# ivan-digital/qwen3-asr-swift

Hardware: NVIDIA B200
Metric: RTFx (audio-sec/sec) Qwen3-ASR-0.6B batched (higher is better)
Workload: dtype bf16

## Files before the change

### qwen3-asr-swift_b200/csrc/api.cu

```cuda
#include <stdio.h>
#include <string.h>

#include <algorithm>
#include <mutex>

#include "gemm.cuh"
#include "model.h"

using namespace q3;

struct q3asr_handle {
    Handle h;
};

namespace {

thread_local std::string g_create_error;

template <typename F>
int guarded(q3asr_handle* hh, F&& fn) {
    if (hh == nullptr) return Q3ASR_ERR_INVALID;
    try {
        DeviceGuard g(hh->h.device);
        fn(hh->h);
// ... 675 lines not shown
        Q3_H2D_SYNC(dseg, seg_row0, sizeof(int) * n_segs);
        Q3_H2D_SYNC(dseg + n_segs, seg_len, sizeof(int) * n_segs);
        Q3_CUDA(cudaMemset(dout, 0, 2 * nq));
        int max_len = 0;
        for (int i = 0; i < n_segs; i++) max_len = std::max(max_len, seg_len[i]);
        AttnSegs segs{dseg, dseg + n_segs, n_segs, max_len};
        cudaError_t se = cudaSuccess;
        try {
            const int ldq = heads * head_dim, ldk = (heads / group) * head_dim;
            if (kernel == 0)
                flash_attn_tc_launch(dq, ldq, dk, ldk, dv, ldk, dout, ldq, segs, rows, heads, group, head_dim, causal != 0, scale, h.stream);
            else
                flash_attn_launch(dq, ldq, dk, ldk, dv, ldk, dout, ldq, segs, heads, group, head_dim, causal != 0, scale, h.stream);
            se = cudaStreamSynchronize(h.stream);
            if (se == cudaSuccess) se = cudaMemcpy(out, dout, 2 * nq, cudaMemcpyDeviceToHost);
        } catch (...) {
            cudaFree(dq); cudaFree(dk); cudaFree(dv); cudaFree(dout); cudaFree(dseg);
            throw;
        }
        cudaFree(dq); cudaFree(dk); cudaFree(dv); cudaFree(dout); cudaFree(dseg);
        Q3_CUDA(se);
    });
}

int q3asr_debug_decode_attention(q3asr_handle* hh, const float* qkv_part, int splits, int n_seqs, int heads, int kv_heads,
                                 const uint16_t* q_norm, const uint16_t* k_norm, float eps, float scale, const int* kv_len,
                                 const int* page_table, int max_pages, uint16_t* pool, int n_pages, int layers, int layer, int variant,
                                 int launches, uint16_t* out) {
    return guarded(hh, [&](Handle& h) {
        Q3_CHECK(h.loaded && h.model, Q3ASR_ERR_STATE, "debug_decode_attention: no model loaded (the RoPE frequencies come from it)");
        Q3_CHECK(qkv_part && q_norm && k_norm && kv_len && page_table && pool && out && splits >= 1 && n_seqs >= 1 && kv_heads >= 1 &&
                     heads >= 1 && max_pages >= 1 && n_pages >= 1 && layers >= 1 && layer >= 0 && layer < layers && launches >= 1,
                 Q3ASR_ERR_INVALID, "debug_decode_attention: bad argument");
        Q3_CHECK(variant == -1 || variant == 0 || variant == 1 || variant == 2 || variant == 4 || variant == 8 || variant == 16,
                 Q3ASR_ERR_INVALID, "debug_decode_attention: variant must be -1, 0, 1, 2, 4, 8 or 16");
        Q3_CHECK(variant == -1 ? (heads == kv_heads || heads == 2 * kv_heads) : heads == 2 * kv_heads, Q3ASR_ERR_INVALID,
                 "debug_decode_attention: the fused kernels take 2 query heads per kv head, the general path 1 or 2");
        for (size_t i = 0; i < (size_t)n_seqs * max_pages; i++)
            Q3_CHECK(page_table[i] >= 0 && page_table[i] < n_pages, Q3ASR_ERR_INVALID, "debug_decode_attention: page-table entry out of range");
        for (int s = 0; s < n_seqs; s++)
            Q3_CHECK(kv_len[s] >= 1 && kv_len[s] <= max_pages * KV_PAGE, Q3ASR_ERR_INVALID, "debug_decode_attention: kv_len out of range");
        const int nqkv = (heads + 2 * kv_heads) * 128, n_pos = max_pages * KV_PAGE;
        const size_t part_n = (size_t)splits * n_seqs * nqkv, out_n = (size_t)n_seqs * heads * 128;
        const size_t pool_n = (size_t)n_pages * layers * 2 * kv_heads * KV_PAGE * 128;
        DebugAllocs a;
        std::vector<int> pos(n_seqs), row_seq(n_seqs);
        for (int s = 0; s < n_seqs; s++) { pos[s] = kv_len[s] - 1; row_seq[s] = s; }
        float* dpart = a.get<float>(part_n);
        bf16 *dqw = a.get<bf16>(128), *dkw = a.get<bf16>(128), *dpool = a.get<bf16>(pool_n), *dout = a.get<bf16>(out_n * launches);
        int *dlen = a.get<int>(n_seqs), *dpos = a.get<int>(n_seqs), *dpt = a.get<int>((size_t)n_seqs * max_pages);
        float2* drope = a.get<float2>((size_t)n_pos * 64);
        Q3_H2D_SYNC(dpart, qkv_part, sizeof(float) * part_n);
        Q3_H2D_SYNC(dqw, q_norm, 2 * 128);
        Q3_H2D_SYNC(dkw, k_norm, 2 * 128);
        Q3_H2D_SYNC(dpool, pool, 2 * pool_n);
        Q3_H2D_SYNC(dlen, kv_len, sizeof(int) * n_seqs);
        Q3_H2D_SYNC(dpos, pos.data(), sizeof(int) * n_seqs);
        Q3_H2D_SYNC(dpt, page_table, sizeof(int) * (size_t)n_seqs * max_pages);
        rope_table_launch(h.model->inv_freq, n_pos, drope, nullptr, h.stream);
        const KvCache cache{dpool, dpt, max_pages, layers, kv_heads, 128};
        if (variant == -1) {
            std::vector<bf16> qkv((size_t)n_seqs * nqkv);
            for (size_t i = 0; i < qkv.size(); i++) {
                float acc = 0.f;
                for (int sp = 0; sp < splits; sp++) acc += qkv_part[(size_t)sp * n_seqs * nqkv + i];
                qkv[i] = __float2bfloat16_rn(acc);
            }
            bf16 *dqkv = a.get<bf16>(qkv.size()), *dq = a.get<bf16>(out_n);
// ... 96 lines not shown
```

### qwen3-asr-swift_b200/csrc/gemm.cu

```cuda
#include <cudaTypedefs.h>
#include <stdlib.h>

#include <atomic>
#include <vector>

#include "gemm2.cuh"
#include "lmhead.cuh"
#include "skinny.cuh"

namespace q3 {

namespace {

PFN_cuTensorMapEncodeTiled_v12000 g_encode = nullptr;
int g_num_sms = 148;
thread_local unsigned long long g_launches = 0;

void make_tmap(CUtensorMap* m, const void* ptr, int rank, const cuuint64_t* dims, const cuuint64_t* strides_bytes,
               const cuuint32_t* box, const cuuint32_t* estr, CUtensorMapSwizzle swizzle = CU_TENSOR_MAP_SWIZZLE_128B) {
    Q3_CHECK(g_encode != nullptr, 2, "gemm_init() has not been called");
    CUresult r = g_encode(m, CU_TENSOR_MAP_DATA_TYPE_BFLOAT16, (cuuint32_t)rank, const_cast<void*>(ptr), dims, strides_bytes, box,
                          estr, CU_TENSOR_MAP_INTERLEAVE_NONE, swizzle, CU_TENSOR_MAP_L2_PROMOTION_L2_256B,
                          CU_TENSOR_MAP_FLOAT_OOB_FILL_NONE);
    if (r != CUDA_SUCCESS) {
        std::string s = "cuTensorMapEncodeTiled failed (" + std::to_string((int)r) + "): rank " + std::to_string(rank) + " dims";
        for (int i = 0; i < rank; i++) s += " " + std::to_string((unsigned long long)dims[i]);
        s += " strides";
        for (int i = 0; i + 1 < rank; i++) s += " " + std::to_string((unsigned long long)strides_bytes[i]);
        s += " box";
        for (int i = 0; i < rank; i++) s += " " + std::to_string(box[i]);
        s += " estr";
        for (int i = 0; i < rank; i++) s += " " + std::to_string(estr[i]);
        throw Error(3, s);
    }
}

template <int BN, int EPI>
void launch_tc(const CUtensorMap& ta, const CUtensorMap& tb, const CUtensorMap& tc, GemmDev p, int max_stages, int grid, cudaStream_t st) {
    static PerDeviceOnce attr_once;
// ... 209 lines not shown
        s_m = mm;
    }
    __syncthreads();
    const float M = s_m;
    float s = 0.f;
    for (int t = threadIdx.x; t < tiles; t += blockDim.x) {
        const float mt = mx[t];
        if (mt != -INFINITY) s += sm[t] * __expf(mt - M);
    }
#pragma unroll
    for (int o = 16; o > 0; o >>= 1) s += __shfl_xor_sync(0xffffffffu, s, o);
    __syncthreads();
    if (lane == 0) sv[warp] = s;
    __syncthreads();
    if (threadIdx.x == 0) {
        float tot = 0.f;
        for (int w = 0; w < 8; w++) tot += sv[w];
        const float z = raw ? __bfloat162float(raw[(size_t)row * ld + bi]) : best;
        out[row] = bi;
        if (out_val) out_val[row] = best;
        out_lp[row] = (z - M) - logf(tot);
    }
}

}

void make_tmap_2d_bf16(CUtensorMap* m, const void* ptr, uint64_t cols, uint64_t rows, uint64_t row_stride_elems, uint32_t box_cols,
                       uint32_t box_rows) {
    cuuint64_t dims[2] = {(cuuint64_t)cols, (cuuint64_t)rows};
    cuuint64_t str[1] = {(cuuint64_t)row_stride_elems * 2};
    cuuint32_t box[2] = {box_cols, box_rows};
    cuuint32_t es[2] = {1, 1};
    make_tmap(m, ptr, 2, dims, str, box, es);
}

void gemm_init(int device) {
    if (g_encode == nullptr) {
        void* fn = nullptr;
        cudaDriverEntryPointQueryResult qres;
        Q3_CUDA(cudaGetDriverEntryPoint("cuTensorMapEncodeTiled", &fn, cudaEnableDefault, &qres));
        Q3_CHECK(qres == cudaDriverEntryPointSuccess && fn != nullptr, 3, "cuTensorMapEncodeTiled not available in this driver");
        g_encode = reinterpret_cast<PFN_cuTensorMapEncodeTiled_v12000>(fn);
    }
    cudaDeviceProp prop;
    Q3_CUDA(cudaGetDeviceProperties(&prop, device));
    Q3_CHECK(prop.major == 10, 3, std::string("q3asr kernels are built for sm_100a only; device is sm_") + std::to_string(prop.major) +
                                      std::to_string(prop.minor));
    g_num_sms = prop.multiProcessorCount;
}

int gemm_pick_bn(int N, int epi, long m_tiles) {
    static const int cand[] = {256, 224, 160, 128, 64, 32};
    int smallest = 0;
    for (int bn : cand) {
        if (N % bn) continue;
        if (epi == EPI_SWIGLU && bn % (2 * GU_UNIT)) continue;
        smallest = bn;
        if (m_tiles * (N / bn) >= 2L * g_num_sms) return bn;
    }
    Q3_CHECK(smallest != 0, 1, "gemm: N = " + std::to_string(N) + " is not a multiple of 32");
    return smallest;
}
int gemm_pick_bn(int N, int epi) { return gemm_pick_bn(N, epi, 1L << 20); }

void gemm_conv(const GemmA& a, const GemmShape& s, const bf16* W, int N, const GemmEpiArgs& e, cudaStream_t st, bool simt, int bn) {
    Q3_CHECK(a.C % 8 == 0 && a.C > 0, 1, "gemm: channel count must be a positive multiple of 8");
// ... 271 lines not shown
```

### qwen3-asr-swift_b200/csrc/ops.cu

```cuda
#include <stdlib.h>

#include <algorithm>

#include "ops.cuh"
#include "ptx.cuh"

namespace q3 {

namespace {

__device__ __forceinline__ uint2 ld8(const bf16* p) { return *reinterpret_cast<const uint2*>(p); }
__device__ __forceinline__ void st8(bf16* p, float a, float b, float c, float d) {
    *reinterpret_cast<uint2*>(p) = make_uint2(pack_bf16x2(a, b), pack_bf16x2(c, d));
}

__global__ void __launch_bounds__(256) conv1_kernel(const float* __restrict__ mel, const Conv1Chunk* __restrict__ chunks,
                                                    const bf16* __restrict__ w, const bf16* __restrict__ bias, int C, int chunk_w,
                                                    bf16* __restrict__ out) {
    extern __shared__ float2 s_in[];
    const int oh = blockIdx.x, g = blockIdx.y;
    const Conv1Chunk c = chunks[g];
    const int pitch = chunk_w + 2;
    for (int i = threadIdx.x; i < 3 * pitch; i += blockDim.x) {
        const int r = i / pitch, j = i % pitch - 1;
// ... 484 lines not shown
        out[((size_t)seq * heads + kvh * GROUP + g) * 128 + d] = __float2bfloat16_rn(num / den);
    }
}

constexpr int DM_CHUNK = 16;
constexpr int DM_STAGES = 3;
constexpr int DM_STREAMS = 8;

__device__ __forceinline__ float dm_merge_scales(float am, float bm, float* fa, float* fb) {
    const float m = fmaxf(am, bm);
    *fa = am == -INFINITY ? 0.f : exp2f(am - m);
    *fb = bm == -INFINITY ? 0.f : exp2f(bm - m);
    return m;
}
constexpr int decode_attn_mma_smem(int nw) { return nw * DM_STAGES * 2 * DM_CHUNK * 128 * 2; }

__device__ __forceinline__ void ldsm_x4(uint32_t (&r)[4], const void* smem_ptr) {
    const uint32_t a = static_cast<uint32_t>(__cvta_generic_to_shared(smem_ptr));
    asm volatile("ldmatrix.sync.aligned.m8n8.x4.shared.b16 {%0,%1,%2,%3}, [%4];" : "=r"(r[0]), "=r"(r[1]), "=r"(r[2]), "=r"(r[3]) : "r"(a));
}
__device__ __forceinline__ void ldsm_x4_t(uint32_t (&r)[4], const void* smem_ptr) {
    const uint32_t a = static_cast<uint32_t>(__cvta_generic_to_shared(smem_ptr));
    asm volatile("ldmatrix.sync.aligned.m8n8.x4.trans.shared.b16 {%0,%1,%2,%3}, [%4];"
                 : "=r"(r[0]), "=r"(r[1]), "=r"(r[2]), "=r"(r[3])
                 : "r"(a));
}
__device__ __forceinline__ void mma16816(float (&d)[4], const uint32_t (&a)[4], uint32_t b0, uint32_t b1) {
    asm volatile("mma.sync.aligned.m16n8k16.row.col.f32.bf16.bf16.f32 {%0,%1,%2,%3}, {%4,%5,%6,%7}, {%8,%9}, {%0,%1,%2,%3};"
                 : "+f"(d[0]), "+f"(d[1]), "+f"(d[2]), "+f"(d[3])
                 : "r"(a[0]), "r"(a[1]), "r"(a[2]), "r"(a[3]), "r"(b0), "r"(b1));
}
__device__ __forceinline__ int dm_off(int key, int seg) { return key * 128 + ((seg ^ (key & 7)) << 3); }

constexpr int DM_PART_STRIDE = 264;
template <int NW, bool SPLIT>
__global__ void __launch_bounds__(NW * 32, SPLIT ? 8 : NW == 2 ? 4 : 1) decode_attn_mma_kernel(const float* __restrict__ qkv_part, int splits, long long split_stride,
                                                                  int nqkv, const bf16* __restrict__ qw, const bf16* __restrict__ kw,
                                                                  const int* __restrict__ pos, float eps,
                                                                  const float2* __restrict__ rope_tab, KvCache cache, int layer,
                                                                  const int* __restrict__ kv_len, int heads, float scale_log2,
                                                                  bf16* __restrict__ out, float* __restrict__ split_part, int* __restrict__ split_cnt) {
    static_assert(!SPLIT || NW == 1, "the split variant is one warp per CTA");
    constexpr int GROUP = 2;
    constexpr int SW = SPLIT ? 2 : NW;
    ptx::grid_dep_launch();
    const int seq = blockIdx.x, kvh = blockIdx.y;
    const int lane = threadIdx.x & 31, warp = threadIdx.x >> 5;
    const int half = SPLIT ? (int)blockIdx.z : 0;
    const int sw0 = SPLIT ? half : warp;
    __shared__ __align__(16) bf16 s_qb[GROUP][128];
    __shared__ __align__(16) bf16 s_new[2][128];
    __shared__ float s_m[GROUP][NW], s_l[GROUP][NW];
    __shared__ float s_acc[GROUP][NW][128];
    const int* pt = cache.page_table + (size_t)seq * cache.max_pages;

    const int len = kv_len[seq];
    extern __shared__ uint4 da_smem[];
    bf16* ring = reinterpret_cast<bf16*>(da_smem) + (size_t)warp * DM_STAGES * 2 * DM_CHUNK * 128;
    const size_t head_off = (((size_t)layer * 2) * cache.kv_heads + kvh) * (KV_PAGE * 128);
    const size_t page_elems = (size_t)cache.layers * 2 * cache.kv_heads * (KV_PAGE * 128);
    const size_t v_off = (size_t)cache.kv_heads * (KV_PAGE * 128);
    const int n_chunks = (len + DM_CHUNK - 1) / DM_CHUNK;
    auto issue = [&](int chunk, int stage) {
        if (chunk < n_chunks) {
            const int j0 = chunk * DM_CHUNK;
            const bf16* kb = cache.pool + (size_t)pt[j0 / KV_PAGE] * page_elems + head_off + (j0 % KV_PAGE) * 128;
            bf16* sk = ring + (size_t)stage * 2 * DM_CHUNK * 128;
#pragma unroll
            for (int i = 0; i < DM_CHUNK * 16 / 32; i++) {
                const int lin = i * 32 + lane, key = lin >> 4, seg = lin & 15;
                const uint32_t n = j0 + key < len ? 16u : 0u;
                cp_async16(sk + dm_off(key, seg), kb + lin * 8, n);
                cp_async16(sk + DM_CHUNK * 128 + dm_off(key, seg), kb + v_off + lin * 8, n);
            }
        }
        asm volatile("cp.async.commit_group;" ::: "memory");
    };
    auto seq_next = [&](int& sj, int& sc) {
        sc += DM_STREAMS;
        while (sc >= n_chunks && sj + SW < DM_STREAMS) {
            sj += SW;
            sc = sj;
        }
    };
    int ij = sw0, ic = sw0;
    while (ic >= n_chunks && ij + SW < DM_STREAMS) { ij += SW; ic = ij; }
#pragma unroll
    for (int s = 0; s < DM_STAGES - 1; s++) {
        issue(ic, s);
        seq_next(ij, ic);
    }

    ptx::grid_dep_wait();

    const bool need_kv = !SPLIT || half == 0 || (((n_chunks - 1) % DM_STREAMS) & 1) == half;
    for (int vt = threadIdx.x; vt < 16 * (GROUP + 2) && (vt < 16 * GROUP || need_kv); vt += NW * 32) {
        const int slot = vt >> 4, hl = vt & 15;
        const unsigned half_mask = 0xffffu << (threadIdx.x & 16);
        const int d0 = hl * 8;
        const int col = slot < GROUP ? (kvh * GROUP + slot) * 128
                                     : slot == GROUP ? heads * 128 + kvh * 128 : (heads + cache.kv_heads) * 128 + kvh * 128;
        const float* src = qkv_part + (size_t)seq * nqkv + col + d0;
        float x[8] = {0.f, 0.f, 0.f, 0.f, 0.f, 0.f, 0.f, 0.f};
        for (int s0 = 0; s0 < splits; s0 += 4) {
            float4 b[4][2];
#pragma unroll
            for (int i = 0; i < 4; i++) {
                const bool on = s0 + i < splits;
                const float4* sp = reinterpret_cast<const float4*>(src + (size_t)(s0 + i) * split_stride);
                b[i][0] = on ? sp[0] : make_float4(0.f, 0.f, 0.f, 0.f);
                b[i][1] = on ? sp[1] : make_float4(0.f, 0.f, 0.f, 0.f);
            }
#pragma unroll
            for (int i = 0; i < 4; i++) {
                x[0] += b[i][0].x; x[1] += b[i][0].y; x[2] += b[i][0].z; x[3] += b[i][0].w;
                x[4] += b[i][1].x; x[5] += b[i][1].y; x[6] += b[i][1].z; x[7] += b[i][1].w;
            }
        }
#pragma unroll
        for (int j = 0; j < 8; j++) x[j] = bf16_round(x[j]);
        const int p = pos[seq];
        if (slot <= GROUP) {
            float q = 0.f;
#pragma unroll
            for (int j = 0; j < 8; j++) q = fmaf(x[j], x[j], q);
#pragma unroll
            for (int o = 8; o > 0; o >>= 1) q += __shfl_xor_sync(half_mask, q, o);
            const float r = rsqrtf(q * (1.0f / 128.0f) + eps);
            const uint4 wu = *reinterpret_cast<const uint4*>((slot < GROUP ? qw : kw) + d0);
            const uint32_t ww[4] = {wu.x, wu.y, wu.z, wu.w};
#pragma unroll
            for (int j = 0; j < 4; j++) {
                const float2 wf = unpack_bf16x2(ww[j]);
                x[2 * j] = bf16_round(x[2 * j] * r * wf.x);
                x[2 * j + 1] = bf16_round(x[2 * j + 1] * r * wf.y);
            }
            float y[8];
#pragma unroll
            for (int j = 0; j < 8; j++) y[j] = __shfl_xor_sync(half_mask, x[j], 8);
            const float sgn = hl < 8 ? -1.f : 1.f;
            const float4* tp = reinterpret_cast<const float4*>(rope_tab + (size_t)p * 64 + (d0 & 63));
#pragma unroll
            for (int j = 0; j < 4; j++) {
                const float4 t = __ldg(tp + j);
                x[2 * j] = fmaf(x[2 * j], t.x, sgn * y[2 * j] * t.y);
                x[2 * j + 1] = fmaf(x[2 * j + 1], t.z, sgn * y[2 * j + 1] * t.w);
            }
        }
        const uint4 packed = make_uint4(pack_bf16x2(x[0], x[1]), pack_bf16x2(x[2], x[3]), pack_bf16x2(x[4], x[5]), pack_bf16x2(x[6], x[7]));
        if (slot < GROUP) {
            *reinterpret_cast<uint4*>(&s_qb[slot][d0]) = packed;
        } else {
            const int page = pt[p / KV_PAGE];
            bf16* dst = cache.pool + ((((size_t)page * cache.layers + layer) * 2 + (slot == GROUP ? 0 : 1)) * cache.kv_heads + kvh) * (KV_PAGE * 128) +
                        (p % KV_PAGE) * 128 + d0;
            if (half == 0) *reinterpret_cast<uint4*>(dst) = packed;
            *reinterpret_cast<uint4*>(&s_new[slot - GROUP][d0]) = packed;
        }
    }
    __syncthreads();

    const int g = lane >> 2, t = lane & 3;
    uint32_t qa[8][2];
#pragma unroll
    for (int ks = 0; ks < 8; ks++) {
        qa[ks][0] = lane < 8 ? *reinterpret_cast<const uint32_t*>(&s_qb[g & 1][ks * 16 + t * 2]) : 0u;
        qa[ks][1] = lane < 8 ? *reinterpret_cast<const uint32_t*>(&s_qb[g & 1][ks * 16 + 8 + t * 2]) : 0u;
    }
    float o[16][4];
    float m_run = -INFINITY, l_run = 0.f;
    const int mi = lane >> 3, r8 = lane & 7;
    int stage = 0;
    int cj = sw0, chunk = sw0;
    while (chunk >= n_chunks && cj + SW < DM_STREAMS) { cj += SW; chunk = cj; }
    int cur_stream = -1;
    bool first_stream = true;
    auto flush_stream = [&]() {
        float l = l_run;
        l += __shfl_xor_sync(0xffffffffu, l, 1);
        l += __shfl_xor_sync(0xffffffffu, l, 2);
        if (lane < 8) {
            float am = first_stream ? -INFINITY : s_m[g][warp], al = first_stream ? 0.f : s_l[g][warp];
            float fa, fb;
            const float mm = dm_merge_scales(am, m_run, &fa, &fb);
#pragma unroll
            for (int nt = 0; nt < 16; nt++) {
                float* dst = &s_acc[g][warp][nt * 8 + t * 2];
                const float a0 = first_stream ? 0.f : dst[0], a1 = first_stream ? 0.f : dst[1];
                dst[0] = fmaf(fb, o[nt][0], fa * a0);
                dst[1] = fmaf(fb, o[nt][1], fa * a1);
            }
            __syncwarp(0xffu);
            if (t == 0) { s_m[g][warp] = mm; s_l[g][warp] = fmaf(fb, l, fa * al); }
        }
        first_stream = false;
    };
    for (; chunk < n_chunks; seq_next(cj, chunk)) {
        if (cj != cur_stream) {
            if (cur_stream >= 0) flush_stream();
            cur_stream = cj;
#pragma unroll
            for (int i = 0; i < 16; i++) o[i][0] = o[i][1] = o[i][2] = o[i][3] = 0.f;
            m_run = -INFINITY;
            l_run = 0.f;
        }
        issue(ic, (stage + DM_STAGES - 1) % DM_STAGES);
        seq_next(ij, ic);
        asm volatile("cp.async.wait_group %0;" ::"n"(DM_STAGES - 1) : "memory");
        __syncwarp();
        bf16* sk = ring + (size_t)stage * 2 * DM_CHUNK * 128;
        bf16* sv = sk + DM_CHUNK * 128;
        const int j0 = chunk * DM_CHUNK;
        if (chunk == n_chunks - 1) {
            const int row = (len - 1) - j0;
            *reinterpret_cast<uint4*>((lane < 16 ? sk : sv) + dm_off(row, lane & 15)) = reinterpret_cast<const uint4*>(s_new[lane >> 4])[lane & 15];
            __syncwarp();
        }
        float s[2][4];
#pragma unroll
        for (int i = 0; i < 2; i++) s[i][0] = s[i][1] = s[i][2] = s[i][3] = 0.f;
#pragma unroll
        for (int ks = 0; ks < 8; ks++) {
            uint32_t b[4];
            const int key = (mi >> 1) * 8 + r8;
            ldsm_x4(b, sk + dm_off(key, ks * 2 + (mi & 1)));
            const uint32_t a[4] = {qa[ks][0], 0u, qa[ks][1], 0u};
            mma16816(s[0], a, b[0], b[1]);
            mma16816(s[1], a, b[2], b[3]);
        }
        float mx = -INFINITY;
#pragma unroll
        for (int nt = 0; nt < 2; nt++)
#pragma unroll
            for (int e = 0; e < 2; e++) {
                const bool ok = j0 + nt * 8 + t * 2 + e < len;
                s[nt][e] = ok ? s[nt][e] * scale_log2 : -INFINITY;
                mx = fmaxf(mx, s[nt][e]);
            }
        mx = fmaxf(mx, __shfl_xor_sync(0xffffffffu, mx, 1));
        mx = fmaxf(mx, __shfl_xor_sync(0xffffffffu, mx, 2));
        const float mn = fmaxf(m_run, mx);
        const float alpha = exp2f(m_run - mn);
        m_run = mn;
        const float p00 = exp2f(s[0][0] - mn), p01 = exp2f(s[0][1] - mn), p10 = exp2f(s[1][0] - mn), p11 = exp2f(s[1][1] - mn);
        l_run = l_run * alpha + ((p00 + p01) + (p10 + p11));
        const uint32_t pa[4] = {pack_bf16x2(p00, p01), 0u, pack_bf16x2(p10, p11), 0u};
#pragma unroll
        for (int i = 0; i < 16; i++) { o[i][0] *= alpha; o[i][1] *= alpha; }
#pragma unroll
        for (int np = 0; np < 8; np++) {
            uint32_t b[4];
            const int key = r8 + (mi & 1) * 8;
            ldsm_x4_t(b, sv + dm_off(key, np * 2 + (mi >> 1)));
            mma16816(o[2 * np], pa, b[0], b[1]);
            mma16816(o[2 * np + 1], pa, b[2], b[3]);
        }
        __syncwarp();
        stage = (stage + 1) % DM_STAGES;
    }
    asm volatile("cp.async.wait_group 0;" ::: "memory");

    if (cur_stream >= 0) {
        flush_stream();
    } else if (lane < 8) {
        if (t == 0) { s_m[g][warp] = -INFINITY; s_l[g][warp] = 0.f; }
#pragma unroll
        for (int nt = 0; nt < 16; nt++) s_acc[g][warp][nt * 8 + t * 2] = s_acc[g][warp][nt * 8 + t * 2 + 1] = 0.f;
    }
    __syncthreads();
    if constexpr (SPLIT) {
        const size_t item = (size_t)seq * gridDim.y + kvh;
        float* mine = split_part + (item * 2 + half) * DM_PART_STRIDE;
        for (int i = lane; i < GROUP * 128; i += 32) mine[i] = s_acc[i >> 7][0][i & 127];
        if (lane < 2 * GROUP) mine[GROUP * 128 + lane] = lane < GROUP ? s_m[lane][0] : s_l[lane - GROUP][0];
        __threadfence();
        __syncwarp();
        int arrived = 0;
        if (lane == 0) arrived = atomicAdd(split_cnt + item, 1);
        arrived = __shfl_sync(0xffffffffu, arrived, 0);
        if (arrived == 0) return;
        __threadfence();
        const float* other = split_part + (item * 2 + (half ^ 1)) * DM_PART_STRIDE;
        for (int i = lane; i < GROUP * 128; i += 32) {
            const int gg = i >> 7, d = i & 127;
            const float om = __ldcg(other + GROUP * 128 + gg), ol = __ldcg(other + GROUP * 128 + GROUP + gg), oa = __ldcg(other + i);
            const float em = half == 0 ? s_m[gg][0] : om, el = half == 0 ? s_l[gg][0] : ol, ea = half == 0 ? s_acc[gg][0][d] : oa;
            const float dm = half == 0 ? om : s_m[gg][0], dl = half == 0 ? ol : s_l[gg][0], da = half == 0 ? oa : s_acc[gg][0][d];
            float fa, fb;
            dm_merge_scales(em, dm, &fa, &fb);
            const float num = fmaf(fb, da, fa * ea), den = fmaf(fb, dl, fa * el);
            out[((size_t)seq * heads + kvh * GROUP + gg) * 128 + d] = __float2bfloat16_rn(num / den);
        }
        if (lane == 0) split_cnt[item] = 0;
    } else
    for (int i = threadIdx.x; i < GROUP * 128; i += NW * 32) {
        const int gg = i >> 7, d = i & 127;
        float cm[2] = {-INFINITY, -INFINITY}, cl[2] = {0.f, 0.f}, ca[2] = {0.f, 0.f};
#pragma unroll
        for (int w = 0; w < NW; w++) {
            float fa, fb;
            const float mm = dm_merge_scales(cm[w & 1], s_m[gg][w], &fa, &fb);
            ca[w & 1] = fmaf(fb, s_acc[gg][w][d], fa * ca[w & 1]);
            cl[w & 1] = fmaf(fb, s_l[gg][w], fa * cl[w & 1]);
            cm[w & 1] = mm;
        }
        float fa, fb;
        dm_merge_scales(cm[0], cm[1], &fa, &fb);
        const float num = fmaf(fb, ca[1], fa * ca[0]), den = fmaf(fb, cl[1], fa * cl[0]);
        out[((size_t)seq * heads + kvh * GROUP + gg) * 128 + d] = __float2bfloat16_rn(num / den);
    }
}

__global__ void __launch_bounds__(1024) reduce_resid_rmsnorm_kernel(const float* __restrict__ part, int splits, long long split_stride,
                                                                    bf16* __restrict__ x, const bf16* __restrict__ w, bf16* __restrict__ y,
                                                                    int d, float eps) {
    ptx::grid_dep_launch();
    ptx::grid_dep_wait();
    __shared__ float4 s_part[1024];
    __shared__ float s_red[32];
    const int ncg = d >> 2, sg_count = blockDim.x / ncg;
    const int row = blockIdx.x, cg = threadIdx.x % ncg, sg = threadIdx.x / ncg, c0 = cg * 4;
    const float* src = part + (size_t)row * d + c0;
    float4 b[4];
#pragma unroll
    for (int i = 0; i < 4; i++) {
        const int sp = sg + i * sg_count;
        b[i] = sp < splits ? *reinterpret_cast<const float4*>(src + (size_t)sp * split_stride) : make_float4(0.f, 0.f, 0.f, 0.f);
    }
    float4 a = b[0];
#pragma unroll
    for (int i = 1; i < 4; i++) { a.x += b[i].x; a.y += b[i].y; a.z += b[i].z; a.w += b[i].w; }
    for (int sp = sg + 4 * sg_count; sp < splits; sp += sg_count) {
        const float4 t = *reinterpret_cast<const float4*>(src + (size_t)sp * split_stride);
        a.x += t.x; a.y += t.y; a.z += t.z; a.w += t.w;
    }
    s_part[threadIdx.x] = a;
    __syncthreads();
    float v[4] = {0.f, 0.f, 0.f, 0.f};
    float q = 0.f;
    if (sg == 0) {
        for (int g = 1; g < sg_count; g++) {
            const float4 t = s_part[g * ncg + cg];
// ... 337 lines not shown
    if (rows <= 0) return;
    launch_kernel(embed_splice_kernel, blocks_for((size_t)rows * (h / 8), 256), 256, 0, st, ids, audio_src, embed, audio, x, rows, h);
}

void qknorm_rope_kv_launch(const bf16* qkv, int ld, const bf16* qw, const bf16* kw, const int* pos, const int* row_seq, int rows,
                           int heads, int kv_heads, float eps, const float2* rope_tab, bf16* qout, bf16* kc, bf16* vc,
                           const KvCache& cache, int layer, cudaStream_t st) {
    if (rows <= 0) return;
    Q3_CHECK(cache.head_dim == 128, 1, "decoder head_dim must be 128");
    qknorm_rope_kv_kernel<<<rows, 256, 0, st>>>(qkv, ld, qw, kw, pos, row_seq, rows, heads, kv_heads, eps, rope_tab, qout,
                                                                kc, vc, cache, layer);
    Q3_CUDA(cudaGetLastError());
}

void rope_table_launch(const float* inv_freq, int n_pos, float2* tab, float2* tab_t, cudaStream_t st) {
    if (n_pos > 0) rope_table_kernel<<<blocks_for((size_t)n_pos * 64, 256), 256, 0, st>>>(inv_freq, n_pos, tab, tab_t);
    Q3_CUDA(cudaGetLastError());
}

void decode_attn_launch(const bf16* q, const KvCache& cache, int layer, const int* kv_len, int n_seqs, int heads, float scale, bf16* out,
                        cudaStream_t st) {
    if (n_seqs <= 0) return;
    const int group = heads / cache.kv_heads;
    const float sl2 = scale * 1.4426950408889634f;
    dim3 grid(n_seqs, cache.kv_heads);
    switch (group) {
        case 1: decode_attn_kernel<1><<<grid, 128, 0, st>>>(q, cache, layer, kv_len, heads, sl2, out); break;
        case 2: decode_attn_kernel<2><<<grid, 128, 0, st>>>(q, cache, layer, kv_len, heads, sl2, out); break;
        default: throw Error(1, "decode attention: only 1 or 2 query heads per kv head are built");
    }
    Q3_CUDA(cudaGetLastError());
}

void decode_attn_fused_launch(const float* qkv_part, int splits, long long split_stride, int nqkv, const bf16* qw, const bf16* kw,
                              const int* pos, float eps, const float2* rope_tab, const KvCache& cache, int layer, const int* kv_len,
                              int n_seqs, int heads, float scale, bf16* out, int num_sms, cudaStream_t st, float* split_part, int* split_cnt,
                              int force) {
    if (n_seqs <= 0) return;
    Q3_CHECK(cache.head_dim == 128, 1, "decoder head_dim must be 128");
    Q3_CHECK(heads == 2 * cache.kv_heads, 1, "fused decode attention is built for 2 query heads per kv head");
    Q3_CHECK(force == 0 || force == 2 || force == 4 || force == 8 || force == 16 || (force == 1 && split_part != nullptr && split_cnt != nullptr), 1,
             "fused decode attention: unknown variant");
    const float sl2 = scale * 1.4426950408889634f;
    dim3 grid(n_seqs, cache.kv_heads);
    static PerDeviceOnce attr_once;
    attr_once([] {
        Q3_CUDA(cudaFuncSetAttribute(decode_attn_fused_kernel<2, 4>, cudaFuncAttributeMaxDynamicSharedMemorySize, decode_attn_smem(4)));
        Q3_CUDA(cudaFuncSetAttribute(decode_attn_fused_kernel<2, 16>, cudaFuncAttributeMaxDynamicSharedMemorySize, decode_attn_smem(16)));
        Q3_CUDA(cudaFuncSetAttribute(decode_attn_mma_kernel<1, true>, cudaFuncAttributeMaxDynamicSharedMemorySize, decode_attn_mma_smem(1)));
        Q3_CUDA(cudaFuncSetAttribute(decode_attn_mma_kernel<2, false>, cudaFuncAttributeMaxDynamicSharedMemorySize, decode_attn_mma_smem(2)));
        Q3_CUDA(cudaFuncSetAttribute(decode_attn_mma_kernel<8, false>, cudaFuncAttributeMaxDynamicSharedMemorySize, decode_attn_mma_smem(8)));
    });
    const long items = (long)n_seqs * cache.kv_heads;
    int warps = items >= 2L * num_sms ? 2 : 8;
    if (const char* f = getenv("Q3ASR_DECODE_ATTN_WARPS")) {
        const int w = atoi(f);
        if (w == 2 || w == 8 || (w == 1 && split_part != nullptr && split_cnt != nullptr)) warps = w;
    }
    static const bool simt_env = getenv("Q3ASR_DECODE_ATTN_SIMT") != nullptr && atoi(getenv("Q3ASR_DECODE_ATTN_SIMT")) != 0;
    bool simt = simt_env;
    if (force != 0) {
        simt = force == 4 || force == 16;
        warps = force == 16 ? 8 : force == 4 ? 2 : force;
    }
    if (!simt) {
        if (warps == 1)
            launch_kernel(decode_attn_mma_kernel<1, true>, dim3(n_seqs, cache.kv_heads, 2), 32, decode_attn_mma_smem(1), st, qkv_part, splits,
                          split_stride, nqkv, qw, kw, pos, eps, rope_tab, cache, layer, kv_len, heads, sl2, out, split_part, split_cnt);
        else if (warps == 2)
            launch_kernel(decode_attn_mma_kernel<2, false>, grid, 64, decode_attn_mma_smem(2), st, qkv_part, splits, split_stride, nqkv, qw, kw, pos, eps,
                          rope_tab, cache, layer, kv_len, heads, sl2, out, split_part, split_cnt);
        else
            launch_kernel(decode_attn_mma_kernel<8, false>, grid, 256, decode_attn_mma_smem(8), st, qkv_part, splits, split_stride, nqkv, qw, kw, pos, eps,
                          rope_tab, cache, layer, kv_len, heads, sl2, out, split_part, split_cnt);
    } else if (warps <= 2) {
        launch_kernel(decode_attn_fused_kernel<2, 4>, grid, 128, decode_attn_smem(4), st, qkv_part, splits, split_stride, nqkv, qw, kw, pos, eps,
                      rope_tab, cache, layer, kv_len, heads, sl2, out);
    } else {
        launch_kernel(decode_attn_fused_kernel<2, 16>, grid, 512, decode_attn_smem(16), st, qkv_part, splits, split_stride, nqkv, qw, kw, pos,
                      eps, rope_tab, cache, layer, kv_len, heads, sl2, out);
    }
}

void reduce_resid_rmsnorm_launch(const float* part, int splits, long long split_stride, bf16* x, const bf16* w, bf16* y, int rows, int d,
                                 float eps, cudaStream_t st) {
    if (rows <= 0) return;
    Q3_CHECK(d % 128 == 0 && d <= 2048, 1, "reduce_resid_rmsnorm: d must be a multiple of 128, <= 2048");
    const int ncg = d / 4;
    int sg = std::max(1, std::min(1024 / ncg, (splits + 3) / 4 > 0 ? 1024 / ncg : 1));
    while (sg > 1 && sg > splits) sg >>= 1;
    launch_kernel(reduce_resid_rmsnorm_kernel, rows, ncg * sg, 0, st, part, splits, split_stride, x, w, y, d, eps);
}

void decode_advance_launch(const DecodeState& s, int n_seqs, cudaStream_t st, bool per_seq) {
    Q3_CHECK(n_seqs <= 1024, 1, "decode_advance: at most 1024 sequences per handle");
    Q3_CHECK(!per_seq || s.slot_seq != nullptr, 1, "decode_advance: per-sequence steps need the row -> sequence map");
    if (per_seq) launch_kernel(decode_advance_kernel<true>, 1, 1024, 0, st, s, n_seqs);
    else launch_kernel(decode_advance_kernel<false>, 1, 1024, 0, st, s, n_seqs);
}
// ... 65 lines not shown
```

Measured before the change: 7763.

## Add persistent TMA-pipelined decode attention kernel for large batches

Adds a persistent decode-attention kernel, one block per SM, that loops over (sequence, kv-head) items. Each consumer warp streams KV chunks through a 3-stage TMA/mbarrier ring built on a new 4D tensor map of the paged KV pool. A producer warp prepares the next item's normed, RoPE'd q/k/v while the current item is consumed. It becomes the default when items >= 2x SMs, replacing the 2-warp mma kernel. The goal is to hide KV load latency and launch/tail effects, at the cost of a per-launch host tensor-map encode and more complex sync.

Result: slower. 6989, median of 6 (-10.0%).

```diff
diff --git a/qwen3-asr-swift_b200/csrc/api.cu b/qwen3-asr-swift_b200/csrc/api.cu
--- a/qwen3-asr-swift_b200/csrc/api.cu
+++ b/qwen3-asr-swift_b200/csrc/api.cu
@@ -731,8 +731,8 @@
         Q3_CHECK(qkv_part && q_norm && k_norm && kv_len && page_table && pool && out && splits >= 1 && n_seqs >= 1 && kv_heads >= 1 &&
                      heads >= 1 && max_pages >= 1 && n_pages >= 1 && layers >= 1 && layer >= 0 && layer < layers && launches >= 1,
                  Q3ASR_ERR_INVALID, "debug_decode_attention: bad argument");
-        Q3_CHECK(variant == -1 || variant == 0 || variant == 1 || variant == 2 || variant == 4 || variant == 8 || variant == 16,
-                 Q3ASR_ERR_INVALID, "debug_decode_attention: variant must be -1, 0, 1, 2, 4, 8 or 16");
+        Q3_CHECK(variant == -1 || variant == 0 || variant == 1 || variant == 2 || variant == 4 || variant == 8 || variant == 9 || variant == 16,
+                 Q3ASR_ERR_INVALID, "debug_decode_attention: variant must be -1, 0, 1, 2, 4, 8, 9 or 16");
         Q3_CHECK(variant == -1 ? (heads == kv_heads || heads == 2 * kv_heads) : heads == 2 * kv_heads, Q3ASR_ERR_INVALID,
                  "debug_decode_attention: the fused kernels take 2 query heads per kv head, the general path 1 or 2");
         for (size_t i = 0; i < (size_t)n_seqs * max_pages; i++)
diff --git a/qwen3-asr-swift_b200/csrc/gemm.cu b/qwen3-asr-swift_b200/csrc/gemm.cu
--- a/qwen3-asr-swift_b200/csrc/gemm.cu
+++ b/qwen3-asr-swift_b200/csrc/gemm.cu
@@ -5,6 +5,7 @@
 #include <vector>
 
 #include "gemm2.cuh"
+#include "ops.cuh"
 #include "lmhead.cuh"
 #include "skinny.cuh"
 
@@ -280,6 +281,15 @@
     cuuint32_t box[2] = {box_cols, box_rows};
     cuuint32_t es[2] = {1, 1};
     make_tmap(m, ptr, 2, dims, str, box, es);
+}
+
+void make_tmap_kv_pool(CUtensorMap* m, const void* pool, int layers, int kv_heads) {
+    const cuuint64_t slab = (cuuint64_t)KV_PAGE * 128 * 2;
+    cuuint64_t dims[4] = {128, (cuuint64_t)KV_PAGE, (cuuint64_t)layers * 2 * kv_heads, 1ull << 24};
+    cuuint64_t str[3] = {128 * 2, slab, slab * layers * 2 * kv_heads};
+    cuuint32_t box[4] = {64, 16, 1, 1};
+    cuuint32_t es[4] = {1, 1, 1, 1};
+    make_tmap(m, pool, 4, dims, str, box, es);
 }
 
 void gemm_init(int device) {
diff --git a/qwen3-asr-swift_b200/csrc/ops.cu b/qwen3-asr-swift_b200/csrc/ops.cu
--- a/qwen3-asr-swift_b200/csrc/ops.cu
+++ b/qwen3-asr-swift_b200/csrc/ops.cu
@@ -540,6 +540,142 @@
 }
 __device__ __forceinline__ int dm_off(int key, int seg) { return key * 128 + ((seg ^ (key & 7)) << 3); }
 
+__device__ __forceinline__ void dm_new_token(int vt, const float* __restrict__ qkv_part, int splits, long long split_stride, int nqkv,
+                                             const bf16* __restrict__ qw, const bf16* __restrict__ kw, const int* __restrict__ pos, float eps,
+                                             const float2* __restrict__ rope_tab, const KvCache& cache, int layer, int heads, int seq, int kvh,
+                                             const int* __restrict__ pt, bool append, bf16 (*s_qb)[128], bf16 (*s_new)[128]) {
+    constexpr int GROUP = 2;
+    const int slot = vt >> 4, hl = vt & 15;
+    const unsigned half_mask = 0xffffu << (threadIdx.x & 16);
+    const int d0 = hl * 8;
+    const int col = slot < GROUP ? (kvh * GROUP + slot) * 128
+                                 : slot == GROUP ? heads * 128 + kvh * 128 : (heads + cache.kv_heads) * 128 + kvh * 128;
+    const float* src = qkv_part + (size_t)seq * nqkv + col + d0;
+    float x[8] = {0.f, 0.f, 0.f, 0.f, 0.f, 0.f, 0.f, 0.f};
+    for (int s0 = 0; s0 < splits; s0 += 4) {
+        float4 b[4][2];
+#pragma unroll
+        for (int i = 0; i < 4; i++) {
+            const bool on = s0 + i < splits;
+            const float4* sp = reinterpret_cast<const float4*>(src + (size_t)(s0 + i) * split_stride);
+            b[i][0] = on ? sp[0] : make_float4(0.f, 0.f, 0.f, 0.f);
+            b[i][1] = on ? sp[1] : make_float4(0.f, 0.f, 0.f, 0.f);
+        }
+#pragma unroll
+        for (int i = 0; i < 4; i++) {
+            x[0] += b[i][0].x; x[1] += b[i][0].y; x[2] += b[i][0].z; x[3] += b[i][0].w;
+            x[4] += b[i][1].x; x[5] += b[i][1].y; x[6] += b[i][1].z; x[7] += b[i][1].w;
+        }
+    }
+#pragma unroll
+    for (int j = 0; j < 8; j++) x[j] = bf16_round(x[j]);
+    const int p = pos[seq];
+    if (slot <= GROUP) {
+        float q = 0.f;
+#pragma unroll
+        for (int j = 0; j < 8; j++) q = fmaf(x[j], x[j], q);
+#pragma unroll
+        for (int o = 8; o > 0; o >>= 1) q += __shfl_xor_sync(half_mask, q, o);
+        const float r = rsqrtf(q * (1.0f / 128.0f) + eps);
+        const uint4 wu = *reinterpret_cast<const uint4*>((slot < GROUP ? qw : kw) + d0);
+        const uint32_t ww[4] = {wu.x, wu.y, wu.z, wu.w};
+#pragma unroll
+        for (int j = 0; j < 4; j++) {
+            const float2 wf = unpack_bf16x2(ww[j]);
+            x[2 * j] = bf16_round(x[2 * j] * r * wf.x);
+            x[2 * j + 1] = bf16_round(x[2 * j + 1] * r * wf.y);
+        }
+        float y[8];
+#pragma unroll
+        for (int j = 0; j < 8; j++) y[j] = __shfl_xor_sync(half_mask, x[j], 8);
+        const float sgn = hl < 8 ? -1.f : 1.f;
+        const float4* tp = reinterpret_cast<const float4*>(rope_tab + (size_t)p * 64 + (d0 & 63));
+#pragma unroll
+        for (int j = 0; j < 4; j++) {
+            const float4 t = __ldg(tp + j);
+            x[2 * j] = fmaf(x[2 * j], t.x, sgn * y[2 * j] * t.y);
+            x[2 * j + 1] = fmaf(x[2 * j + 1], t.z, sgn * y[2 * j + 1] * t.w);
+        }
+    }
+    const uint4 packed = make_uint4(pack_bf16x2(x[0], x[1]), pack_bf16x2(x[2], x[3]), pack_bf16x2(x[4], x[5]), pack_bf16x2(x[6], x[7]));
+    if (slot < GROUP) {
+        *reinterpret_cast<uint4*>(&s_qb[slot][d0]) = packed;
+    } else {
+        const int page = pt[p / KV_PAGE];
+        bf16* dst = cache.pool + ((((size_t)page * cache.layers + layer) * 2 + (slot == GROUP ? 0 : 1)) * cache.kv_heads + kvh) * (KV_PAGE * 128) +
+                    (p % KV_PAGE) * 128 + d0;
+        if (append) *reinterpret_cast<uint4*>(dst) = packed;
+        *reinterpret_cast<uint4*>(&s_new[slot - GROUP][d0]) = packed;
+    }
+}
+
+template <class Off>
+__device__ __forceinline__ void dm_chunk(const bf16* sk, const bf16* sv, Off off, const uint32_t (&qa)[8][2], int j0, int len, float scale_log2,
+                                         float (&o)[16][4], float& m_run, float& l_run) {
+    const int lane = threadIdx.x & 31;
+    const int t = lane & 3, mi = lane >> 3, r8 = lane & 7;
+    float s[2][4];
+#pragma unroll
+    for (int i = 0; i < 2; i++) s[i][0] = s[i][1] = s[i][2] = s[i][3] = 0.f;
+#pragma unroll
+    for (int ks = 0; ks < 8; ks++) {
+        uint32_t b[4];
+        const int key = (mi >> 1) * 8 + r8;
+        ldsm_x4(b, sk + off(key, ks * 2 + (mi & 1)));
+        const uint32_t a[4] = {qa[ks][0], 0u, qa[ks][1], 0u};
+        mma16816(s[0], a, b[0], b[1]);
+        mma16816(s[1], a, b[2], b[3]);
+    }
+    float mx = -INFINITY;
+#pragma unroll
+    for (int nt = 0; nt < 2; nt++)
+#pragma unroll
+        for (int e = 0; e < 2; e++) {
+            const bool ok = j0 + nt * 8 + t * 2 + e < len;
+            s[nt][e] = ok ? s[nt][e] * scale_log2 : -INFINITY;
+            mx = fmaxf(mx, s[nt][e]);
+        }
+    mx = fmaxf(mx, __shfl_xor_sync(0xffffffffu, mx, 1));
+    mx = fmaxf(mx, __shfl_xor_sync(0xffffffffu, mx, 2));
+    const float mn = fmaxf(m_run, mx);
+    const float alpha = exp2f(m_run - mn);
+    m_run = mn;
+    const float p00 = exp2f(s[0][0] - mn), p01 = exp2f(s[0][1] - mn), p10 = exp2f(s[1][0] - mn), p11 = exp2f(s[1][1] - mn);
+    l_run = l_run * alpha + ((p00 + p01) + (p10 + p11));
+    const uint32_t pa[4] = {pack_bf16x2(p00, p01), 0u, pack_bf16x2(p10, p11), 0u};
+#pragma unroll
+    for (int i = 0; i < 16; i++) { o[i][0] *= alpha; o[i][1] *= alpha; }
+#pragma unroll
+    for (int np = 0; np < 8; np++) {
+        uint32_t b[4];
+        const int key = r8 + (mi & 1) * 8;
+        ldsm_x4_t(b, sv + off(key, np * 2 + (mi >> 1)));
+        mma16816(o[2 * np], pa, b[0], b[1]);
+        mma16816(o[2 * np + 1], pa, b[2], b[3]);
+    }
+}
+
+template <int NW>
+__device__ __forceinline__ void dm_merge_store(const float (*s_m)[NW], const float (*s_l)[NW], const float (*s_acc)[NW][128], bf16* __restrict__ out) {
+    constexpr int GROUP = 2;
+    for (int i = threadIdx.x; i < GROUP * 128; i += NW * 32) {
+        const int gg = i >> 7, d = i & 127;
+        float cm[2] = {-INFINITY, -INFINITY}, cl[2] = {0.f, 0.f}, ca[2] = {0.f, 0.f};
+#pragma unroll
+        for (int w = 0; w < NW; w++) {
+            float fa, fb;
+            const float mm = dm_merge_scales(cm[w & 1], s_m[gg][w], &fa, &fb);
+            ca[w & 1] = fmaf(fb, s_acc[gg][w][d], fa * ca[w & 1]);
+            cl[w & 1] = fmaf(fb, s_l[gg][w], fa * cl[w & 1]);
+            cm[w & 1] = mm;
+        }
+        float fa, fb;
+        dm_merge_scales(cm[0], cm[1], &fa, &fb);
+        const float num = fmaf(fb, ca[1], fa * ca[0]), den = fmaf(fb, cl[1], fa * cl[0]);
+        out[i] = __float2bfloat16_rn(num / den);
+    }
+}
+
 constexpr int DM_PART_STRIDE = 264;
 template <int NW, bool SPLIT>
 __global__ void __launch_bounds__(NW * 32, SPLIT ? 8 : NW == 2 ? 4 : 1) decode_attn_mma_kernel(const float* __restrict__ qkv_part, int splits, long long split_stride,
@@ -602,70 +738,8 @@
     ptx::grid_dep_wait();
 
     const bool need_kv = !SPLIT || half == 0 || (((n_chunks - 1) % DM_STREAMS) & 1) == half;
-    for (int vt = threadIdx.x; vt < 16 * (GROUP + 2) && (vt < 16 * GROUP || need_kv); vt += NW * 32) {
-        const int slot = vt >> 4, hl = vt & 15;
-        const unsigned half_mask = 0xffffu << (threadIdx.x & 16);
-        const int d0 = hl * 8;
-        const int col = slot < GROUP ? (kvh * GROUP + slot) * 128
-                                     : slot == GROUP ? heads * 128 + kvh * 128 : (heads + cache.kv_heads) * 128 + kvh * 128;
-        const float* src = qkv_part + (size_t)seq * nqkv + col + d0;
-        float x[8] = {0.f, 0.f, 0.f, 0.f, 0.f, 0.f, 0.f, 0.f};
-        for (int s0 = 0; s0 < splits; s0 += 4) {
-            float4 b[4][2];
-#pragma unroll
-            for (int i = 0; i < 4; i++) {
-                const bool on = s0 + i < splits;
-                const float4* sp = reinterpret_cast<const float4*>(src + (size_t)(s0 + i) * split_stride);
-                b[i][0] = on ? sp[0] : make_float4(0.f, 0.f, 0.f, 0.f);
-                b[i][1] = on ? sp[1] : make_float4(0.f, 0.f, 0.f, 0.f);
-            }
-#pragma unroll
-            for (int i = 0; i < 4; i++) {
-                x[0] += b[i][0].x; x[1] += b[i][0].y; x[2] += b[i][0].z; x[3] += b[i][0].w;
-                x[4] += b[i][1].x; x[5] += b[i][1].y; x[6] += b[i][1].z; x[7] += b[i][1].w;
-            }
-        }
-#pragma unroll
-        for (int j = 0; j < 8; j++) x[j] = bf16_round(x[j]);
-        const int p = pos[seq];
-        if (slot <= GROUP) {
-            float q = 0.f;
-#pragma unroll
-            for (int j = 0; j < 8; j++) q = fmaf(x[j], x[j], q);
-#pragma unroll
-            for (int o = 8; o > 0; o >>= 1) q += __shfl_xor_sync(half_mask, q, o);
-            const float r = rsqrtf(q * (1.0f / 128.0f) + eps);
-            const uint4 wu = *reinterpret_cast<const uint4*>((slot < GROUP ? qw : kw) + d0);
-            const uint32_t ww[4] = {wu.x, wu.y, wu.z, wu.w};
-#pragma unroll
-            for (int j = 0; j < 4; j++) {
-                const float2 wf = unpack_bf16x2(ww[j]);
-                x[2 * j] = bf16_round(x[2 * j] * r * wf.x);
-                x[2 * j + 1] = bf16_round(x[2 * j + 1] * r * wf.y);
-            }
-            float y[8];
-#pragma unroll
-            for (int j = 0; j < 8; j++) y[j] = __shfl_xor_sync(half_mask, x[j], 8);
-            const float sgn = hl < 8 ? -1.f : 1.f;
-            const float4* tp = reinterpret_cast<const float4*>(rope_tab + (size_t)p * 64 + (d0 & 63));
-#pragma unroll
-            for (int j = 0; j < 4; j++) {
-                const float4 t = __ldg(tp + j);
-                x[2 * j] = fmaf(x[2 * j], t.x, sgn * y[2 * j] * t.y);
-                x[2 * j + 1] = fmaf(x[2 * j + 1], t.z, sgn * y[2 * j + 1] * t.w);
-            }
-        }
-        const uint4 packed = make_uint4(pack_bf16x2(x[0], x[1]), pack_bf16x2(x[2], x[3]), pack_bf16x2(x[4], x[5]), pack_bf16x2(x[6], x[7]));
-        if (slot < GROUP) {
-            *reinterpret_cast<uint4*>(&s_qb[slot][d0]) = packed;
-        } else {
-            const int page = pt[p / KV_PAGE];
-            bf16* dst = cache.pool + ((((size_t)page * cache.layers + layer) * 2 + (slot == GROUP ? 0 : 1)) * cache.kv_heads + kvh) * (KV_PAGE * 128) +
-                        (p % KV_PAGE) * 128 + d0;
-            if (half == 0) *reinterpret_cast<uint4*>(dst) = packed;
-            *reinterpret_cast<uint4*>(&s_new[slot - GROUP][d0]) = packed;
-        }
-    }
+    for (int vt = threadIdx.x; vt < 16 * (GROUP + 2) && (vt < 16 * GROUP || need_kv); vt += NW * 32)
+        dm_new_token(vt, qkv_part, splits, split_stride, nqkv, qw, kw, pos, eps, rope_tab, cache, layer, heads, seq, kvh, pt, half == 0, s_qb, s_new);
     __syncthreads();
 
     const int g = lane >> 2, t = lane & 3;
@@ -677,7 +751,6 @@
     }
     float o[16][4];
     float m_run = -INFINITY, l_run = 0.f;
-    const int mi = lane >> 3, r8 = lane & 7;
     int stage = 0;
     int cj = sw0, chunk = sw0;
     while (chunk >= n_chunks && cj + SW < DM_STREAMS) { cj += SW; chunk = cj; }
@@ -724,45 +797,7 @@
             *reinterpret_cast<uint4*>((lane < 16 ? sk : sv) + dm_off(row, lane & 15)) = reinterpret_cast<const uint4*>(s_new[lane >> 4])[lane & 15];
             __syncwarp();
         }
-        float s[2][4];
-#pragma unroll
-        for (int i = 0; i < 2; i++) s[i][0] = s[i][1] = s[i][2] = s[i][3] = 0.f;
-#pragma unroll
-        for (int ks = 0; ks < 8; ks++) {
-            uint32_t b[4];
-            const int key = (mi >> 1) * 8 + r8;
-            ldsm_x4(b, sk + dm_off(key, ks * 2 + (mi & 1)));
-            const uint32_t a[4] = {qa[ks][0], 0u, qa[ks][1], 0u};
-            mma16816(s[0], a, b[0], b[1]);
-            mma16816(s[1], a, b[2], b[3]);
-        }
-        float mx = -INFINITY;
-#pragma unroll
-        for (int nt = 0; nt < 2; nt++)
-#pragma unroll
-            for (int e = 0; e < 2; e++) {
-                const bool ok = j0 + nt * 8 + t * 2 + e < len;
-                s[nt][e] = ok ? s[nt][e] * scale_log2 : -INFINITY;
-                mx = fmaxf(mx, s[nt][e]);
-            }
-        mx = fmaxf(mx, __shfl_xor_sync(0xffffffffu, mx, 1));
-        mx = fmaxf(mx, __shfl_xor_sync(0xffffffffu, mx, 2));
-        const float mn = fmaxf(m_run, mx);
-        const float alpha = exp2f(m_run - mn);
-        m_run = mn;
-        const float p00 = exp2f(s[0][0] - mn), p01 = exp2f(s[0][1] - mn), p10 = exp2f(s[1][0] - mn), p11 = exp2f(s[1][1] - mn);
-        l_run = l_run * alpha + ((p00 + p01) + (p10 + p11));
-        const uint32_t pa[4] = {pack_bf16x2(p00, p01), 0u, pack_bf16x2(p10, p11), 0u};
-#pragma unroll
-        for (int i = 0; i < 16; i++) { o[i][0] *= alpha; o[i][1] *= alpha; }
-#pragma unroll
-        for (int np = 0; np < 8; np++) {
-            uint32_t b[4];
-            const int key = r8 + (mi & 1) * 8;
-            ldsm_x4_t(b, sv + dm_off(key, np * 2 + (mi >> 1)));
-            mma16816(o[2 * np], pa, b[0], b[1]);
-            mma16816(o[2 * np + 1], pa, b[2], b[3]);
-        }
+        dm_chunk(sk, sv, dm_off, qa, j0, len, scale_log2, o, m_run, l_run);
         __syncwarp();
         stage = (stage + 1) % DM_STAGES;
     }
@@ -801,21 +836,141 @@
         }
         if (lane == 0) split_cnt[item] = 0;
     } else
-    for (int i = threadIdx.x; i < GROUP * 128; i += NW * 32) {
-        const int gg = i >> 7, d = i & 127;
-        float cm[2] = {-INFINITY, -INFINITY}, cl[2] = {0.f, 0.f}, ca[2] = {0.f, 0.f};
-#pragma unroll
-        for (int w = 0; w < NW; w++) {
-            float fa, fb;
-            const float mm = dm_merge_scales(cm[w & 1], s_m[gg][w], &fa, &fb);
-            ca[w & 1] = fmaf(fb, s_acc[gg][w][d], fa * ca[w & 1]);
-            cl[w & 1] = fmaf(fb, s_l[gg][w], fa * cl[w & 1]);
-            cm[w & 1] = mm;
-        }
-        float fa, fb;
-        dm_merge_scales(cm[0], cm[1], &fa, &fb);
-        const float num = fmaf(fb, ca[1], fa * ca[0]), den = fmaf(fb, cl[1], fa * cl[0]);
-        out[((size_t)seq * heads + kvh * GROUP + gg) * 128 + d] = __float2bfloat16_rn(num / den);
+    dm_merge_store<NW>(s_m, s_l, s_acc, out + ((size_t)seq * heads + kvh * GROUP) * 128);
+}
+
+constexpr int DP_WARPS = DM_STREAMS;
+constexpr int DP_THREADS = DP_WARPS * 32 + 32;
+constexpr int DP_STAGES = 3;
+constexpr int DP_SLOT = 2 * DM_CHUNK * 128;
+constexpr int decode_attn_persist_smem() { return DP_WARPS * DP_STAGES * DP_SLOT * 2 + 1024; }
+__device__ __forceinline__ int dp_off(int key, int seg) { return (seg >> 3) * (DM_CHUNK * 64) + key * 64 + (((seg & 7) ^ (key & 7)) << 3); }
+
+__global__ void __launch_bounds__(DP_THREADS, 1) decode_attn_persist_kernel(const float* __restrict__ qkv_part, int splits, long long split_stride,
+                                                                             int nqkv, const bf16* __restrict__ qw, const bf16* __restrict__ kw,
+                                                                             const int* __restrict__ pos, float eps,
+                                                                             const float2* __restrict__ rope_tab, KvCache cache, int layer,
+                                                                             const int* __restrict__ kv_len, int heads, float scale_log2,
+                                                                             bf16* __restrict__ out, int n_seqs,
+                                                                             const __grid_constant__ CUtensorMap tm_pool) {
+    constexpr int GROUP = 2;
+    ptx::grid_dep_launch();
+    const int lane = threadIdx.x & 31, warp = threadIdx.x >> 5;
+    __shared__ __align__(16) bf16 s_qb[2][GROUP][128];
+    __shared__ __align__(16) bf16 s_new[2][2][128];
+    __shared__ float s_m[2][GROUP][DP_WARPS], s_l[2][GROUP][DP_WARPS];
+    __shared__ float s_acc[2][GROUP][DP_WARPS][128];
+    __shared__ __align__(8) uint64_t s_full[DP_WARPS][DP_STAGES];
+    extern __shared__ uint4 da_smem[];
+    bf16* ring = reinterpret_cast<bf16*>((reinterpret_cast<uintptr_t>(da_smem) + 1023) & ~uintptr_t(1023)) + (size_t)warp * DP_STAGES * DP_SLOT;
+    const int kv_heads = cache.kv_heads, n_items = n_seqs * kv_heads;
+    const bool consumer = warp < DP_WARPS;
+    if (consumer && lane == 0) {
+        if (warp == 0) ptx::prefetch_tmap(&tm_pool);
+#pragma unroll
+        for (int i = 0; i < DP_STAGES; i++) ptx::mbar_init(&s_full[warp][i], 1);
+        ptx::fence_barrier_init();
+    }
+    __syncwarp();
+
+    auto n_chunks_of = [&](int item) { return (kv_len[item / kv_heads] + DM_CHUNK - 1) / DM_CHUNK; };
+    int ii = blockIdx.x, ic = warp;
+    auto next = [&]() {
+        ic += DM_STREAMS;
+        while (ii < n_items && ic >= n_chunks_of(ii)) { ii += gridDim.x; ic = warp; }
+    };
+    auto issue = [&](int slot) {
+        if (lane == 0) {
+            const int seq = ii / kv_heads, kvh = ii - seq * kv_heads, j0 = ic * DM_CHUNK;
+            const int page = cache.page_table[(size_t)seq * cache.max_pages + j0 / KV_PAGE], slab = layer * 2 * kv_heads + kvh;
+            bf16* dst = ring + (size_t)slot * DP_SLOT;
+            uint64_t* bar = &s_full[warp][slot];
+            ptx::mbar_arrive_expect_tx(bar, DP_SLOT * 2);
+#pragma unroll
+            for (int i = 0; i < 4; i++)
+                ptx::tma_load_4d(dst + i * (DM_CHUNK * 64), &tm_pool, (i & 1) * 64, j0 % KV_PAGE, slab + (i >> 1) * kv_heads, page, bar);
+        }
+        next();
+    };
+    if (consumer) {
+        ic -= DM_STREAMS;
+        next();
+#pragma unroll
+        for (int i = 0; i < DP_STAGES; i++)
+            if (ii < n_items) issue(i);
+    }
+
+    ptx::grid_dep_wait();
+
+    auto prepare = [&](int item, int b) {
+        const int seq = item / kv_heads, kvh = item - seq * kv_heads;
+        for (int vt = lane; vt < 16 * (GROUP + 2); vt += 32)
+            dm_new_token(vt, qkv_part, splits, split_stride, nqkv, qw, kw, pos, eps, rope_tab, cache, layer, heads, seq, kvh,
+                         cache.page_table + (size_t)seq * cache.max_pages, true, s_qb[b], s_new[b]);
+    };
+    if (!consumer) prepare(blockIdx.x, 0);
+    __syncthreads();
+
+    uint32_t used = 0;
+    const int g = lane >> 2, t = lane & 3;
+    int b = 0;
+    for (int item = blockIdx.x; item < n_items; item += gridDim.x, b ^= 1) {
+        const int seq = item / kv_heads, kvh = item - seq * kv_heads;
+        const int len = kv_len[seq], n_chunks = (len + DM_CHUNK - 1) / DM_CHUNK;
+        if (!consumer) {
+            if (item + (int)gridDim.x < n_items) prepare(item + gridDim.x, b ^ 1);
+        } else {
+        uint32_t qa[8][2];
+#pragma unroll
+        for (int ks = 0; ks < 8; ks++) {
+            qa[ks][0] = lane < 8 ? *reinterpret_cast<const uint32_t*>(&s_qb[b][g & 1][ks * 16 + t * 2]) : 0u;
+            qa[ks][1] = lane < 8 ? *reinterpret_cast<const uint32_t*>(&s_qb[b][g & 1][ks * 16 + 8 + t * 2]) : 0u;
+        }
+        float o[16][4];
+#pragma unroll
+        for (int i = 0; i < 16; i++) o[i][0] = o[i][1] = o[i][2] = o[i][3] = 0.f;
+        float m_run = -INFINITY, l_run = 0.f;
+        for (int chunk = warp; chunk < n_chunks; chunk += DM_STREAMS, used++) {
+            const int slot = used % DP_STAGES;
+            ptx::mbar_wait(&s_full[warp][slot], (used / DP_STAGES) & 1);
+            bf16* sk = ring + (size_t)slot * DP_SLOT;
+            bf16* sv = sk + DM_CHUNK * 128;
+            const int j0 = chunk * DM_CHUNK;
+            const bool last = chunk == n_chunks - 1;
+            if (last) {
+                const int row = (len - 1) - j0;
+                for (int rr = row + 1; rr < DM_CHUNK; rr++) *reinterpret_cast<uint4*>((lane < 16 ? sk : sv) + dp_off(rr, lane & 15)) = make_uint4(0u, 0u, 0u, 0u);
+                *reinterpret_cast<uint4*>((lane < 16 ? sk : sv) + dp_off(row, lane & 15)) = reinterpret_cast<const uint4*>(s_new[b][lane >> 4])[lane & 15];
+                __syncwarp();
+            }
+            dm_chunk(sk, sv, dp_off, qa, j0, len, scale_log2, o, m_run, l_run);
+            if (last) ptx::fence_proxy_async();
+            __syncwarp();
+            if (ii < n_items) issue(slot);
+        }
+        float l = l_run;
+        l += __shfl_xor_sync(0xffffffffu, l, 1);
+        l += __shfl_xor_sync(0xffffffffu, l, 2);
+        if (lane < 8) {
+            if (warp < n_chunks) {
+                float fa, fb;
+                const float mm = dm_merge_scales(-INFINITY, m_run, &fa, &fb);
+#pragma unroll
+                for (int nt = 0; nt < 16; nt++) {
+                    float* dst = &s_acc[b][g][warp][nt * 8 + t * 2];
+                    dst[0] = fmaf(fb, o[nt][0], fa * 0.f);
+                    dst[1] = fmaf(fb, o[nt][1], fa * 0.f);
+                }
+                if (t == 0) { s_m[b][g][warp] = mm; s_l[b][g][warp] = fmaf(fb, l, fa * 0.f); }
+            } else {
+                if (t == 0) { s_m[b][g][warp] = -INFINITY; s_l[b][g][warp] = 0.f; }
+#pragma unroll
+                for (int nt = 0; nt < 16; nt++) s_acc[b][g][warp][nt * 8 + t * 2] = s_acc[b][g][warp][nt * 8 + t * 2 + 1] = 0.f;
+            }
+        }
+        }
+        __syncthreads();
+        dm_merge_store<DP_WARPS>(s_m[b], s_l[b], s_acc[b], out + ((size_t)seq * heads + kvh * GROUP) * 128);
     }
 }
 
@@ -1219,6 +1374,8 @@
     Q3_CUDA(cudaGetLastError());
 }
 
+void make_tmap_kv_pool(CUtensorMap* m, const void* pool, int layers, int kv_heads);
+
 void decode_attn_fused_launch(const float* qkv_part, int splits, long long split_stride, int nqkv, const bf16* qw, const bf16* kw,
                               const int* pos, float eps, const float2* rope_tab, const KvCache& cache, int layer, const int* kv_len,
                               int n_seqs, int heads, float scale, bf16* out, int num_sms, cudaStream_t st, float* split_part, int* split_cnt,
@@ -1226,8 +1383,9 @@
     if (n_seqs <= 0) return;
     Q3_CHECK(cache.head_dim == 128, 1, "decoder head_dim must be 128");
     Q3_CHECK(heads == 2 * cache.kv_heads, 1, "fused decode attention is built for 2 query heads per kv head");
-    Q3_CHECK(force == 0 || force == 2 || force == 4 || force == 8 || force == 16 || (force == 1 && split_part != nullptr && split_cnt != nullptr), 1,
-             "fused decode attention: unknown variant");
+    Q3_CHECK(force == 0 || force == 2 || force == 4 || force == 8 || force == 9 || force == 16 ||
+                 (force == 1 && split_part != nullptr && split_cnt != nullptr),
+             1, "fused decode attention: unknown variant");
     const float sl2 = scale * 1.4426950408889634f;
     dim3 grid(n_seqs, cache.kv_heads);
     static PerDeviceOnce attr_once;
@@ -1237,12 +1395,13 @@
         Q3_CUDA(cudaFuncSetAttribute(decode_attn_mma_kernel<1, true>, cudaFuncAttributeMaxDynamicSharedMemorySize, decode_attn_mma_smem(1)));
         Q3_CUDA(cudaFuncSetAttribute(decode_attn_mma_kernel<2, false>, cudaFuncAttributeMaxDynamicSharedMemorySize, decode_attn_mma_smem(2)));
         Q3_CUDA(cudaFuncSetAttribute(decode_attn_mma_kernel<8, false>, cudaFuncAttributeMaxDynamicSharedMemorySize, decode_attn_mma_smem(8)));
+        Q3_CUDA(cudaFuncSetAttribute(decode_attn_persist_kernel, cudaFuncAttributeMaxDynamicSharedMemorySize, decode_attn_persist_smem()));
     });
     const long items = (long)n_seqs * cache.kv_heads;
-    int warps = items >= 2L * num_sms ? 2 : 8;
+    int warps = items >= 2L * num_sms ? 9 : 8;
     if (const char* f = getenv("Q3ASR_DECODE_ATTN_WARPS")) {
         const int w = atoi(f);
-        if (w == 2 || w == 8 || (w == 1 && split_part != nullptr && split_cnt != nullptr)) warps = w;
+        if (w == 2 || w == 8 || w == 9 || (w == 1 && split_part != nullptr && split_cnt != nullptr)) warps = w;
     }
     static const bool simt_env = getenv("Q3ASR_DECODE_ATTN_SIMT") != nullptr && atoi(getenv("Q3ASR_DECODE_ATTN_SIMT")) != 0;
     bool simt = simt_env;
@@ -1251,7 +1410,12 @@
         warps = force == 16 ? 8 : force == 4 ? 2 : force;
     }
     if (!simt) {
-        if (warps == 1)
+        if (warps == 9) {
+            CUtensorMap tm;
+            make_tmap_kv_pool(&tm, cache.pool, cache.layers, cache.kv_heads);
+            launch_kernel(decode_attn_persist_kernel, (unsigned)std::min<long>(items, num_sms), DP_THREADS, decode_attn_persist_smem(), st, qkv_part,
+                          splits, split_stride, nqkv, qw, kw, pos, eps, rope_tab, cache, layer, kv_len, heads, sl2, out, n_seqs, tm);
+        } else if (warps == 1)
             launch_kernel(decode_attn_mma_kernel<1, true>, dim3(n_seqs, cache.kv_heads, 2), 32, decode_attn_mma_smem(1), st, qkv_part, splits,
                           split_stride, nqkv, qw, kw, pos, eps, rope_tab, cache, layer, kv_len, heads, sl2, out, split_part, split_cnt);
         else if (warps == 2)
```
